# Dane-ME/keypoint-detection

Measured on AMD Instinct MI355X. Metric: images/sec @ 256x192 COCO-17 (MultiPersonKeypointModel.forward, given boxes), higher is better.
Workload: dtype fp32; 1 GPU; C2: batch 64/GPU, 256x192x3, 1 box/img, heatmap head + soft-argmax decode; model=MultiPersonKeypointModel (MobileNetV3-Small+FPN, HeatmapHead), global_batch=64, height=256, width=192, persons=1, precision=split, parallelism=dp1, streams_per_gpu=1, gather=False, gather_pipelined=False

## Files before the change

### keypoint-detection_amd/csrc/conv_glds.hip

```cpp
#include <algorithm>
#include <type_traits>

#include "kpd_common.h"
#include "kpd_kernels.h"
#include "conv_epilogue.h"
#include "kpd_dma.h"

namespace {

typedef _Float16 f16x8 __attribute__((ext_vector_type(8)));
typedef __attribute__((address_space(3))) void lds_void;

constexpr int BM = 256, NT = 512, ROWB = 128;
constexpr unsigned OOB = 0x80000000u;

__device__ __forceinline__ void stamp16(unsigned long long* st, int i, unsigned long long v = 0, int row = -1) {
  if (st && threadIdx.x == 0)
    st[(size_t)(row < 0 ? blockIdx.x : row) * 8 + i] = v ? v : __builtin_amdgcn_s_memrealtime();
}

__device__ __forceinline__ float dpp_xor1(float x) {
  return __int_as_float(__builtin_amdgcn_mov_dpp(__float_as_int(x), 0xB1, 0xF, 0xF, true));
}
__device__ __forceinline__ float dpp_xor2(float x) {
// ... 828 lines not shown
  const int c = (int)(i - px * c8n) * 8, n = (int)(px / hw);
  int a_f, a_l, P;
  fpn0x_exps(sc[(size_t)n * kAmaxStride], sc[(size_t)(N + n) * kAmaxStride], w_exp0, w_expE, &a_f, &a_l, &P);
  const float s = ldexpf(1.f, which ? a_l : a_f);
  const float4 u = *reinterpret_cast<const float4*>(in + px * cin + c);
  const float4 v = *reinterpret_cast<const float4*>(in + px * cin + c + 4);
  const float x[8] = {u.x, u.y, u.z, u.w, v.x, v.y, v.z, v.w};
  typedef _Float16 f16x8v __attribute__((ext_vector_type(8)));
  f16x8v hi, lo;
#pragma unroll
  for (int e = 0; e < 8; ++e) {
    const float xs = x[e] * s;
    hi[e] = (_Float16)xs;
    lo[e] = (_Float16)(xs - (float)hi[e]);
  }
  _Float16* o = out + px * 2 * cin + (c / G) * 2 * G + c % G;
  *reinterpret_cast<f16x8v*>(o) = hi;
  *reinterpret_cast<f16x8v*>(o + G) = lo;
}

constexpr int HP = kHmPitch, HPP = kHmRoiPos;
constexpr int HMS = 56;
constexpr int AWIN = 384;
template <int BMH>
constexpr int hm_awin() { return BMH + 128 <= AWIN ? AWIN : BMH + 128; }
template <int BMH>
constexpr int hm_epi_parts() { return BMH > 256 ? 2 : 1; }
template <int CIN, bool SPLIT>
constexpr int hm_nab() { return (CIN > 0 && (SPLIT ? CIN * 4 : CIN * 2) == 128) ? 1 : 2; }
template <int BMH>
constexpr int kh_epi_parts() { return BMH > 128 ? 2 : 1; }
template <int BN, int BMH>
constexpr int kh_epi_bytes() { return BMH / kh_epi_parts<BMH>() * ((BN + 4) + 68) * 4; }
template <int BN, int SB, int BMH, bool SPLIT, int TPS, int NW, int MODE, int NAB = 2>
constexpr int hmconv_lds_bytes() {
  constexpr int EMODE = MODE >= 0 ? MODE : (BN == 64 ? 1 : 0);
  constexpr int RING = NAB * hm_awin<BMH>() * ROWB + SB * BN * ROWB * TPS;
  constexpr int EPI = EMODE == 2 ? (BN == 128 ? kh_epi_bytes<BN, BMH>() : 0)
                      : EMODE != 0 && EMODE != 3 ? 0 : epi_lds_bytes<BMH / hm_epi_parts<BMH>(), 128, NW * 64>();
  return RING > EPI ? RING : EPI;
}

template <int BMH>
constexpr int hm_pst_stores() { return 2 * 2 * ((BMH / 2 + 31) / 32) * 2; }
template <int BN, int SB, int DBG, int BMH, bool SPLIT, int CIN, int TPS, bool DB, int NW, int MODE, int NTAP,
          bool PST = false>
__device__ __forceinline__ void hmconv_tile(const HmConvArgs& p, char* lds, const int L, const int m_off,
                                            const bool pre = false, const int next_m0 = -1) {
  constexpr int NTH = NW * 64;
  constexpr int EMODE = MODE >= 0 ? MODE : (BN == 64 ? 1 : 0);
  static_assert(NTAP == 9 || (NTAP == 10 && EMODE == 2 && SPLIT && !DB), "tenth tap: KH downsample");
  static_assert(EMODE != 2 || (SPLIT && !DB), "KH epilogue: split, single fragment set");
  constexpr int WAVES_N = BN / 64, WAVES_M = NW / WAVES_N;
  constexpr int WM = BMH / WAVES_M, FM = WM / 16, FN = 4;
  constexpr int AW = hm_awin<BMH>();
  static_assert(WM % 16 == 0 && BMH + 128 <= AW && AW % (8 * NW) == 0, "tile rows");
  static_assert(NW == 8 || (BN == 64 && SPLIT && DB), "4 waves: the conv 3 split DB variant only");
  constexpr int A_LD = AW / 8 / NW;
  static_assert(A_LD <= 9 || TPS > 1, "window pieces: one per tap");
  constexpr int B_LD = BN / 8 / NW;
  constexpr int ABUF = AW * ROWB, BSTAGE = BN * ROWB * TPS;
  static_assert(TPS == 1 || (SPLIT && NTAP % TPS == 0), "taps per step");
  constexpr bool FINAL = EMODE == 1;
  constexpr int NAB = hm_nab<CIN, SPLIT>();
  static_assert(hmconv_lds_bytes<BN, SB, BMH, SPLIT, TPS, NW, MODE, NAB>() <= 160 * 1024, "LDS budget");
  static_assert(!PST || NAB == 2, "persistent tiles: two window buffers");
  static_assert(!PST || (SPLIT && EMODE == 0 && SB == 2 && TPS == 1 && !DB && NW == 8 && NTAP == 9 && BN == 256 &&
                         BMH <= 224 && DBG == 0), "persistent tiles: split conv 1 / conv 2 (BN = cout = 256)");
  auto a_at = [&](int c) { return PST ? (c & 1) * (ABUF + BSTAGE) : NAB == 1 ? 0 : (c & 1) * ABUF; };
  auto b_at = [&](int st) { return PST ? st * (ABUF + BSTAGE) + ABUF : NAB * ABUF + st * BSTAGE; };

  int tid = threadIdx.x;
  if constexpr (PST) asm volatile("" : "+v"(tid));
  const int lane = tid & 63, wave = tid >> 6;
  const int wm = EMODE == 2 ? wave % WAVES_M : wave / WAVES_N, wn = EMODE == 2 ? wave / WAVES_M : wave % WAVES_N;
  const int NTL = p.cout / BN;
  const int m0 = HP + m_off + (L / NTL) * BMH, n0 = (L % NTL) * BN;
  if (m0 >= p.R * HPP) return;
  const int Mtot = p.R * HPP, cin = CIN ? CIN : p.cin, RB = SPLIT ? cin * 4 : cin * 2, NC = RB / 128, KT = NTAP * NC;
  stamp16(p.stamps, 0);
  const int wbase = max(m0 - 64, 0);
  const i32x4 rin = make_rsrc(static_cast<const char*>(p.in) + (size_t)wbase * RB,
                              (int)min(((long)Mtot - wbase) * RB, 0x7fffffffL));
  const i32x4 rwt = make_rsrc(p.wt, p.wt_bytes);
  const unsigned lds0 = (unsigned)reinterpret_cast<unsigned long long>((lds_void*)lds);
  const int lrow = lane >> 3, lchunk = (lane & 7) ^ lrow;
  unsigned a_off[A_LD];
#pragma unroll
// ... 90 lines not shown
  const int KS = KT / TPS;
  if (!PST || !pre) {
#pragma unroll
    for (int i = 0; i < A_LD; ++i) issue_a(0, i);
#pragma unroll
    for (int k = 0; k < SB - 1; ++k)
      if (k < KS) issue_b(k);
    barrier_k(KS < SB - 1);
  } else {
    if (p.amax_idx >= 0) wait_vmcnt<hm_pst_stores<224>() + 2>();
    else wait_vmcnt<hm_pst_stores<224>()>();
    __builtin_amdgcn_s_waitcnt(0xC07F);
    __builtin_amdgcn_s_barrier();
    asm volatile("" ::: "memory");
  }
  stamp16(p.stamps, 1);
  stamp16(p.stamps, 6, __builtin_amdgcn_s_memtime());
  auto issue_a_at = [&](int k1) {
    const int s1 = k1 * TPS, c1 = s1 / NTAP, jj = (s1 - c1 * NTAP) / TPS;
    if (c1 + 1 >= NC) return;
    if constexpr (TPS == 1) {
      if (jj < A_LD) issue_a(c1 + 1, jj);
    } else {
      constexpr int NST = 9 / TPS;
#pragma unroll
      for (int i = 0; i < A_LD; ++i)
        if (i >= jj * A_LD / NST && i < (jj + 1) * A_LD / NST) issue_a(c1 + 1, i);
    }
  };
  issue_a_at(0);
  if (SB - 1 < KS) issue_b(SB - 1);
  auto issue_at = [&](int k1) {
    if constexpr ((DBG & 2) == 0) {
      issue_a_at(k1);
      if (k1 + SB - 1 < KS) issue_b(k1 + SB - 1);
    }
  };
  if constexpr (!SPLIT) {
    Half f0, f1;
    load_half(0, 0, f0);
    for (int k = 0; k < KT; ++k) {
      load_half(k, 1, f1);
      __builtin_amdgcn_s_setprio(1);
      mma_half(f0);
      __builtin_amdgcn_s_setprio(0);
      if (k + 1 < KT) {
        const int k1 = k + 1;
        barrier_k(k1 + SB - 2 >= KT);
        issue_at(k1);
        load_half(k1, 0, f0);
// ... 10 lines not shown
      const int c = k / NTAP, t = k - c * NTAP, off = t == 9 ? 0 : (t / 3 - 1) * HP + (t % 3 - 1);
      const char* ab = lds + a_at(c);
      const int r0w = wm * WM + r16 + 64 + off;
      const int ach = (((q ? 4 : 0) + g) ^ (r0w & 7)) << 4;
#pragma unroll
      for (int i = 0; i < FM; ++i) f[i] = *reinterpret_cast<const uint4*>(ab + (r0w + i * 16) * ROWB + ach);
    };
    const bool late = p.stagger && __builtin_amdgcn_readfirstlane(wave) >= 4;
    auto pass = [&](f32x4 (&A)[FM][FN], const uint4* a, const uint4* b) {
      if constexpr ((DBG & 1) != 0) {
        A[0][0][0] += __uint_as_float(a[0].x ^ b[FN - 1].w);
        return;
      }
      __builtin_amdgcn_s_setprio(1);
#pragma unroll
      for (int i = 0; i < FM; ++i)
#pragma unroll
        for (int j = 0; j < FN; ++j)
          A[i][j] = __builtin_amdgcn_mfma_f32_16x16x32_f16(__builtin_bit_cast(f16x8, a[i]), __builtin_bit_cast(f16x8, b[j]),
                                                           A[i][j], 0, 0, 0);
      __builtin_amdgcn_s_setprio(0);
    };
    if constexpr (DB) {
      static_assert(SB == 2 && 9 % TPS == 0, "DB loop: 2-stage ring");
      int aoff[9];
#pragma unroll
      for (int t = 0; t < 9; ++t) {
        const int r0w = wm * WM + r16 + 64 + (t / 3 - 1) * HP + (t % 3 - 1);
        aoff[t] = r0w * ROWB + ((g ^ (r0w & 7)) << 4);
      }
      struct Frag { uint4 ah[FM], al[FM], bh[FN], bl[FN]; };
      auto rd_all = [&](int c, int t, int stage, Frag& f) {
        const char* ab = lds + a_at(c);
        const char* bb = lds + b_at(stage) + (t % TPS) * BN * ROWB + b_row;
#pragma unroll
        for (int i = 0; i < FM; ++i) {
          f.al[i] = *reinterpret_cast<const uint4*>(ab + (aoff[t] ^ 64) + i * 16 * ROWB);
          f.ah[i] = *reinterpret_cast<const uint4*>(ab + aoff[t] + i * 16 * ROWB);
        }
#pragma unroll
        for (int j = 0; j < FN; ++j) {
          f.bh[j] = *reinterpret_cast<const uint4*>(bb + j * 16 * ROWB + bch0);
          f.bl[j] = *reinterpret_cast<const uint4*>(bb + j * 16 * ROWB + bch1);
        }
      };
      Frag f0, f1;
      rd_all(0, 0, 0, f0);
      for (int c = 0; c < NC; c += 2) {
#pragma unroll
        for (int tt = 0; tt < 18; ++tt) {
          const int cc = c + tt / 9, t = tt % 9, k = cc * 9 + t;
          Frag& cur = (tt & 1) ? f1 : f0;
          Frag& nxt = (tt & 1) ? f0 : f1;
          pass(acc, cur.al, cur.bh);
          const bool kstep = k + 1 < KT && (t + 1) % TPS == 0;
          if (k + 1 < KT) {
            const int tn = (tt + 1) % 18, cn = c + (tt + 1) / 9;
            if (kstep) {
              const int k1 = (k + 1) / TPS;
              barrier_k(k1 + SB - 2 >= KS);
              if (!late) issue_at(k1);
            }
            rd_all(cn, tn % 9, ((tn / 9) * (9 / TPS) + (tn % 9) / TPS) & 1, nxt);
          }
          pass(acc, cur.ah, cur.bh);
          if (kstep && late) issue_at((k + 1) / TPS);
          pass(acc, cur.ah, cur.bl);
        }
      }
    } else {
    auto run_loop = [&](auto NBc, auto NMc, auto NM9c) {
      constexpr int NB_ = decltype(NBc)::value;
      auto rd_bn = [&](int k, int q, uint4* f) {
        const char* bb = lds + b_at((k / TPS) % SB) + (k % TPS) * BN * ROWB;
#pragma unroll
        for (int j = 0; j < NB_; ++j)
          f[j] = *reinterpret_cast<const uint4*>(bb + b_row + j * 16 * ROWB + (q ? bch1 : bch0));
      };
      auto passn = [&](f32x4 (&A)[FM][FN], const uint4* a, const uint4* b, auto NMx) {
        constexpr int NM_ = decltype(NMx)::value;
        if constexpr (NM_ == FN) {
          pass(A, a, b);
        } else if constexpr (NM_ > 0) {
          if constexpr ((DBG & 1) != 0) {
            A[0][0][0] += __uint_as_float(a[0].x ^ b[0].w);
            return;
// ... 442 lines not shown
            char* ob = static_cast<char*>(p.out) + (size_t)m * (p.ns * 4) + (co >> 5) * 128 + (co & 31) * 2;
            *reinterpret_cast<f16x4*>(ob) = hi;
            *reinterpret_cast<f16x4*>(ob + 64) = lo;
          } else {
            *reinterpret_cast<float4*>(p.outf + ((size_t)r * HMS * HMS + yy * HMS + xx) * p.nf +
                                       (co - p.ns)) = make_float4(o[0], o[1], o[2], o[3]);
          }
        }
      }
  
    }
  }
  if (p.stamps) {
    asm volatile("s_waitcnt vmcnt(0)" ::: "memory");
    stamp16(p.stamps, 3);
    stamp16(p.stamps, 5, (unsigned long long)KT);
  }
}

template <int BN, int SB, int DBG = 0, int BMH = BM, bool SPLIT = false, int CIN = 0, int TPS = 1, bool DB = false,
          int NW = 8, int MODE = -1, int NTAP = 9>
__global__ __launch_bounds__(NW * 64) void hmconv_kernel(const HmConvArgs p) {
  __shared__ __attribute__((aligned(1024))) char lds[hmconv_lds_bytes<BN, SB, BMH, SPLIT, TPS, NW, MODE,
                                                                      hm_nab<CIN, SPLIT>()>()];
  hmconv_tile<BN, SB, DBG, BMH, SPLIT, CIN, TPS, DB, NW, MODE, NTAP>(p, lds, xcd_remap(blockIdx.x, gridDim.x),
                                                                        p.m_off);
}

template <typename T>
__device__ __forceinline__ void kernarg_copy(T& dst) {
  typedef const __attribute__((address_space(4))) unsigned* KaPtr;
  KaPtr ka = (KaPtr)__builtin_amdgcn_kernarg_segment_ptr();
  asm volatile("" : "+s"(ka));
  static_assert(sizeof(T) % 4 == 0, "argument block");
  unsigned* d = reinterpret_cast<unsigned*>(&dst);
#pragma unroll
  for (int i = 0; i < (int)(sizeof(T) / 4); ++i) d[i] = ka[i];
}

template <int CIN>
__global__ __launch_bounds__(512) void hmconv_persist_kernel(const HmConvArgs p) {
  __shared__ __attribute__((aligned(1024))) char lds[hmconv_lds_bytes<256, 2, 224, true, 1, 8, -1>()];
  const int G = gridDim.x, w = xcd_remap(blockIdx.x, G);
  const int F = p.mix_F, H = p.mix_H, tail_off = p.m_off + F * 224;
  bool pre = false;
  for (int t = w; t < F; t += G) {
    HmConvArgs pl;
// ... 249 lines not shown
      m.mix_lead = ncu / 16;
      g = dim3((unsigned)(m.mix_F + m.mix_H));
    };
    if (fin && !dbg && !no_tail && !a.stamps && (!split || (a.cin == 256 && hm_db))) {
      const long nfull = rows / BM, F = nfull / ncu * ncu, rem = rows - F * BM, H = (rem + 127) / 128;
      if (split && mix_ok(F, H)) {
        HmConvArgs m = a;
        dim3 g;
        mix_set(m, F, H, g);
        hipLaunchKernelGGL((hmconv_mixed_kernel<64, 2, BM, 128, 256, 3, true, -1>), g, dim3(NT), 0, st, m);
        const hipError_t e = hipGetLastError();
        if (e != hipSuccess) return e;
        continue;
      }
      if (F > 0 && H > 0 && H <= ncu) {
        const dim3 g1((unsigned)F), g2((unsigned)H);
        HmConvArgs a2 = a;
        a2.m_off = (int)(F * BM);
        if (split && hm3_nw4) {
          hipLaunchKernelGGL((hmconv_kernel<64, 2, 0, BM, true, 256, 3, true, 4>), g1, dim3(256), 0, st, a);
          hipLaunchKernelGGL((hmconv_kernel<64, 2, 0, 128, true, 256, 3, true, 4>), g2, dim3(256), 0, st, a2);
        } else if (split) {
          hipLaunchKernelGGL((hmconv_kernel<64, 2, 0, BM, true, 256, 3, true>), g1, dim3(NT), 0, st, a);
          hipLaunchKernelGGL((hmconv_kernel<64, 2, 0, 128, true, 256, 3, true>), g2, dim3(NT), 0, st, a2);
        } else {
          hipLaunchKernelGGL((hmconv_kernel<64, 4>), g1, dim3(NT), 0, st, a);
          hipLaunchKernelGGL((hmconv_kernel<64, 4, 0, 128>), g2, dim3(NT), 0, st, a2);
        }
        const hipError_t e = hipGetLastError();
        if (e != hipSuccess) return e;
        continue;
      }
    }
    static const bool no_tail12 = kpd_diag_env("KPD_HM12_NOTAIL") != nullptr;
#if KPD_DIAG
    static const int persist_env = kpd_diag_env("KPD_HM_PERSIST") ? atoi(kpd_diag_env("KPD_HM_PERSIST")) : 0;
    if (split && !fin && bn == 256 && bm == 224 && a.cout == 256 && (a.cin == 64 || a.cin == 256) && !dbg &&
        !a.stamps && persist_env) {
      const long F = rows / 224 / ncu * ncu, rem = rows - F * 224, H = (rem + 191) / 192;
      if (F > 0 && H <= ncu && F + H < 0x7fffffffL / 224) {
        HmConvArgs m = a;
        m.mix_F = (int)F;
        m.mix_H = (int)H;
        if (a.cin == 64) hipLaunchKernelGGL((hmconv_persist_kernel<64>), dim3((unsigned)ncu), dim3(NT), 0, st, m);
        else hipLaunchKernelGGL((hmconv_persist_kernel<256>), dim3((unsigned)ncu), dim3(NT), 0, st, m);
        const hipError_t e = hipGetLastError();
        if (e != hipSuccess) return e;
// ... 184 lines not shown
```

### keypoint-detection_amd/csrc/head_kernels.hip

```cpp
#include <algorithm>

#include "kpd_common.h"
#include "kpd_kernels.h"

namespace {
constexpr int HM = 56;
static_assert(HM % 4 == 0, "hm_spool / hm_sapply take 4 pixels per load instruction");
constexpr int HMP = HM * HM;
constexpr int NK = 17;
constexpr int TOPK = 64;
constexpr int FC = 128;

__device__ __forceinline__ void slotmap_image(const float* __restrict__ boxes, int b, int P, int32_t* __restrict__ slot);
__global__ __launch_bounds__(256) void topk_kernel(const float* __restrict__ stats, int tiles, int HW,
                                                   const float* __restrict__ w0, const float* __restrict__ b0,
                                                   const float* __restrict__ w2, const float* __restrict__ b2,
                                                   int32_t* __restrict__ topk, float* __restrict__ scores_out,
                                                   const float* __restrict__ boxes, int P, int32_t* __restrict__ slot,
                                                   float* __restrict__ imax, float* __restrict__ sc_zero, int sc_n) {
  extern __shared__ __attribute__((aligned(16))) float tsm[];
  float* sw0 = tsm;
  float* sw2 = sw0 + 8 * FC;
  __shared__ float avg[FC], mx[FC], h[16], sc[FC];
  const int n = blockIdx.x, tid = threadIdx.x, c = tid;
// ... 610 lines not shown
      const float ov[4] = {o.x * ssc, o.y * ssc, o.z * ssc, o.w * ssc};
      f16x4 hi, lo;
#pragma unroll
      for (int e = 0; e < 4; ++e) {
        hi[e] = (_Float16)ov[e];
        lo[e] = (_Float16)(ov[e] - (float)hi[e]);
      }
      _Float16* ob = reinterpret_cast<_Float16*>(xs) + opix * 2 * TOPK + (c >> 3) * 64 + (c & 7) * 4;
      *reinterpret_cast<f16x4*>(ob) = hi;
      *reinterpret_cast<f16x4*>(ob + 32) = lo;
    } else if (out_bf16) {
      const size_t opix = out_bf16 == 2 ? hm_pos(r, y, px)
                                        : ((size_t)r * HM + y) * HM + px;
      bf16x4 ob;
      ob[0] = (__bf16)o.x; ob[1] = (__bf16)o.y; ob[2] = (__bf16)o.z; ob[3] = (__bf16)o.w;
      *reinterpret_cast<bf16x4*>(reinterpret_cast<__bf16*>(xs) + opix * TOPK + 4 * c) = ob;
    } else {
      reinterpret_cast<float4*>(reinterpret_cast<float*>(xs) + (((size_t)r * HM + y) * HM + px) * TOPK)[c] = o;
    }
  }
}

constexpr int kAttBR = 8;
__global__ __launch_bounds__(512) void hm_attn_kernel(const float* __restrict__ roi, const float* __restrict__ cw,
                                                      const float* __restrict__ saw, const float* __restrict__ sab,
                                                      void* __restrict__ xs, int out_bf16, const float* __restrict__ hsc,
                                                      int use_sp, float* __restrict__ sw_out) {
  constexpr int NI = HM / 4, BR = kAttBR, PR = BR + 6;
  __shared__ float w[98];
  __shared__ float2 pool[PR][HM + 6];
  __shared__ float ssw[BR][HM];
  const int nb = HM / BR;
  const int nblk = gridDim.x, L = blockIdx.x;
  const int qx = nblk / 8, rx = nblk % 8, x8 = L % 8, k8 = L / 8;
  const int g = (x8 < rx ? x8 * (qx + 1) : rx * (qx + 1) + (x8 - rx) * qx) + k8;
  const int r = g / nb, y0 = (g - r * nb) * BR;
  const int tid = threadIdx.x, lane = tid & 63, wave = tid >> 6, pp = lane >> 4, c = lane & 15;
  const float4 cq = reinterpret_cast<const float4*>(cw + (size_t)r * TOPK)[c];
  if (tid < 98) w[tid] = saw[tid];
  for (int i = tid; i < PR * 6; i += 512) {
    const int rr = i / 6, cc = i - rr * 6;
    pool[rr][cc < 3 ? cc : HM + cc] = make_float2(0.f, 0.f);
  }
  for (int pr = wave; pr < PR; pr += 8) {
    const int y = y0 - 3 + pr;
    if (y < 0 || y >= HM) {
      if (lane < HM) pool[pr][lane + 3] = make_float2(0.f, 0.f);
      continue;
    }
    const float4* src = reinterpret_cast<const float4*>(roi + ((size_t)r * HM + y) * HM * TOPK);
    float4 v[NI];
#pragma unroll
    for (int i = 0; i < NI; ++i) v[i] = src[(4 * i + pp) * (TOPK / 4) + c];
#pragma unroll
    for (int i = 0; i < NI; ++i) {
      const float a = v[i].x * cq.x, b = v[i].y * cq.y, cc = v[i].z * cq.z, d = v[i].w * cq.w;
      float sm = (a + b) + (cc + d), m = fmaxf(fmaxf(a, b), fmaxf(cc, d));
      sm += dpp_f<0xB1>(sm); m = fmaxf(m, dpp_f<0xB1>(m));
      sm += dpp_f<0x4E>(sm); m = fmaxf(m, dpp_f<0x4E>(m));
      sm += dpp_f<0x124>(sm); m = fmaxf(m, dpp_f<0x124>(m));
      sm += dpp_f<0x128>(sm); m = fmaxf(m, dpp_f<0x128>(m));
      if (c == 0) pool[pr][4 * i + pp + 3] = make_float2(sm / (float)TOPK, m);
    }
  }
  __syncthreads();
  if (tid < BR * HM) {
    const int j = tid / HM, x = tid - j * HM, y = y0 + j;
    float a = 0.f;
#pragma unroll
    for (int ky = 0; ky < 7; ++ky) {
      const int iy = y + ky - 3;
      if (iy < 0 || iy >= HM) continue;
#pragma unroll
      for (int kx = 0; kx < 7; ++kx) {
        const int ix = x + kx - 3;
        if (ix < 0 || ix >= HM) continue;
        const float2 sv2 = pool[j + ky][x + kx];
        a = fmaf(w[ky * 7 + kx], sv2.x, a);
        a = fmaf(w[49 + ky * 7 + kx], sv2.y, a);
      }
    }
    ssw[j][x] = use_sp ? kpd_sigmoid(a + sab[0]) : 1.f;
    if (sw_out) sw_out[((size_t)r * HM + y) * HM + x] = ssw[j][x];
  }
  const float ssc = out_bf16 == 3 ? ldexpf(1.f, split_exp_of(hsc[(size_t)r * 4])) : 1.f;
  __syncthreads();
  {
    const int j = wave, y = y0 + j;
    const float4* src = reinterpret_cast<const float4*>(roi + ((size_t)r * HM + y) * HM * TOPK);
    float4 v[NI];
#pragma unroll
    for (int i = 0; i < NI; ++i) v[i] = src[(4 * i + pp) * (TOPK / 4) + c];
#pragma unroll
    for (int i = 0; i < NI; ++i) {
      const int px = 4 * i + pp;
      const float sw = ssw[j][px];
      const float4 o = make_float4((v[i].x * cq.x) * sw, (v[i].y * cq.y) * sw, (v[i].z * cq.z) * sw, (v[i].w * cq.w) * sw);
      if (out_bf16 == 3) {
        const size_t opix = hm_pos(r, y, px);
        const float ov[4] = {o.x * ssc, o.y * ssc, o.z * ssc, o.w * ssc};
        f16x4 hi, lo;
#pragma unroll
        for (int e = 0; e < 4; ++e) {
          hi[e] = (_Float16)ov[e];
          lo[e] = (_Float16)(ov[e] - (float)hi[e]);
        }
        _Float16* ob = reinterpret_cast<_Float16*>(xs) + opix * 2 * TOPK + (c >> 3) * 64 + (c & 7) * 4;
        *reinterpret_cast<f16x4*>(ob) = hi;
        *reinterpret_cast<f16x4*>(ob + 32) = lo;
      } else if (out_bf16) {
        const size_t opix = out_bf16 == 2 ? hm_pos(r, y, px)
                                          : ((size_t)r * HM + y) * HM + px;
        bf16x4 ob;
        ob[0] = (__bf16)o.x; ob[1] = (__bf16)o.y; ob[2] = (__bf16)o.z; ob[3] = (__bf16)o.w;
        *reinterpret_cast<bf16x4*>(reinterpret_cast<__bf16*>(xs) + opix * TOPK + 4 * c) = ob;
      } else {
        reinterpret_cast<float4*>(reinterpret_cast<float*>(xs) + (((size_t)r * HM + y) * HM + px) * TOPK)[c] = o;
      }
    }
  }
}

__global__ __launch_bounds__(64) void hm_final_kernel(const float* __restrict__ h3, const float* __restrict__ w,
                                                      const float* __restrict__ b, const int32_t* __restrict__ slot,
                                                      int P, float* __restrict__ heat_out) {
  __shared__ float sw[NK * TOPK];
  __shared__ float sb[NK];
  const int y = blockIdx.x, r = blockIdx.y, x = threadIdx.x;
// ... 130 lines not shown
  const size_t lds = std::max<size_t>((size_t)cap * 4, kRoiKhLds);
  hipLaunchKernelGGL(roi_kh_kernel, dim3(HM, R), dim3(256), lds, st, feat, Hf, Wf, topk, boxes, P, roi, roi_stats,
                     cap, static_cast<const _Float16*>(w1s), w1_exp, b1, w2, b2, bound, bdiv, bstride, hsc,
                     static_cast<_Float16*>(out), stamps);
  return hipGetLastError();
}
hipError_t launch_hm_chattn(const float* roi_stats, int R, const float* w0, const float* b0, const float* w2,
                            const float* b2, float* cw, float* hsc, hipStream_t st, int abs_in) {
  hipLaunchKernelGGL(hm_chattn_kernel, dim3(R), dim3(64), 0, st, roi_stats, w0, b0, w2, b2, cw, hsc, abs_in);
  return hipGetLastError();
}
hipError_t launch_hm_spool(const float* roi, const float* cw, int R, float* smap, hipStream_t st) {
  hipLaunchKernelGGL(hm_spool_kernel, dim3(HM, R), dim3(64), 0, st, roi, cw, smap);
  return hipGetLastError();
}
hipError_t launch_hm_sapply(const float* roi, const float* cw, const float* smap, const float* saw,
                            const float* sab, int R, void* xs, int out_bf16, hipStream_t st, const float* hsc,
                            int use_sp, float* sw_out) {
  hipLaunchKernelGGL(hm_sapply_kernel, dim3(HM, R), dim3(64), 0, st, roi, cw, smap, saw, sab, xs, out_bf16, hsc,
                     use_sp, sw_out);
  return hipGetLastError();
}
hipError_t launch_hm_attn(const float* roi, const float* cw, const float* saw, const float* sab, int R, void* xs,
                          int out_bf16, hipStream_t st, const float* hsc, int use_sp, float* sw_out) {
  static_assert(HM % kAttBR == 0 && kAttBR == 8, "one wave per band row");
  if (R <= 0) return hipSuccess;
  hipLaunchKernelGGL(hm_attn_kernel, dim3((unsigned)(R * (HM / kAttBR))), dim3(512), 0, st, roi, cw, saw, sab, xs,
                     out_bf16, hsc, use_sp, sw_out);
  return hipGetLastError();
}
hipError_t launch_hm_final(const float* h3, int R, const float* w, const float* b, const int32_t* slot, int P,
                           float* heat_out, hipStream_t st) {
  hipLaunchKernelGGL(hm_final_kernel, dim3(HM, R), dim3(64), 0, st, h3, w, b, slot, P, heat_out);
  return hipGetLastError();
}
hipError_t launch_decode(const float* heat_out, const float* boxes, const int32_t* slot, int R, int P,
                         float* kpts_out, float* vis_out, hipStream_t st) {
  hipLaunchKernelGGL(decode_kernel, dim3(R, NK), dim3(64), 0, st, heat_out, boxes, slot, P, kpts_out, vis_out);
  return hipGetLastError();
}
```

### keypoint-detection_amd/csrc/kpd_kernels.h

```cpp
#pragma once
#include <hip/hip_runtime.h>
#include <stdint.h>
#include <vector>

struct ConvArgs {
  const void* in;
  const void* wt;
  const float* bias;
  void* out;
  const float* res;
  const float* a_scale;
  float* stats;
  int N, H, W;
  int cin_p, cout_p;
  int in_cstride, out_cstride;
  int rh, rw;
  int act;
  int M;
  int tiles_per_img;
  float* amax;
  const float* post_scale;
  const float* post_shift;
  int act2, act3;
  int in_bytes, wt_bytes;
// ... 202 lines not shown
size_t lateral_chain_lds_bytes(const LatChainArgs& a);
bool lateral_chain_ok(const LatChainArgs& a);
hipError_t launch_lateral_chain(const LatChainArgs& a, int N, hipStream_t st);
hipError_t launch_lateral_stream(const float* in, int cin_p, const float* w, const float* bias, const float* res,
                                 int N, int H, int W, int rh, int rw, void* out, hipStream_t st);

hipError_t launch_topk(const float* stats, int N, int tiles, int HW, const float* w0, const float* b0,
                       const float* w2, const float* b2, int32_t* topk, float* scores, hipStream_t st,
                       const float* boxes = nullptr, int P = 0, int32_t* slot = nullptr, float* imax = nullptr,
                       float* sc_zero = nullptr, int sc_n = 0);
hipError_t launch_slotmap(const float* boxes, int B, int P, int32_t* slot,
                          hipStream_t st);
hipError_t launch_roi_kh(const float* feat, int Hf, int Wf, const int32_t* topk, const float* boxes, int R, int P,
                        float* roi, float* roi_stats, const void* w1s, int w1_exp, const float* b1, const float* w2,
                        const float* b2, const float* bound, int bdiv, int bstride, float* hsc, void* out,
                        hipStream_t st, unsigned long long* stamps = nullptr);
hipError_t launch_roi_align(const float* feat, int Hf, int Wf, int Cf, const int32_t* topk,
                            const float* boxes, int R, int P, float* roi, float* roi_stats,
                            hipStream_t st, unsigned long long* stamps = nullptr);
hipError_t launch_hm_chattn(const float* roi_stats, int R, const float* w0, const float* b0,
                            const float* w2, const float* b2, float* cw, float* hsc, hipStream_t st,
                            int abs_in = 0);
hipError_t launch_hm_spool(const float* roi, const float* cw, int R, float* smap, hipStream_t st);
hipError_t launch_hm_attn(const float* roi, const float* cw, const float* saw, const float* sab, int R, void* xs,
                          int out_bf16, hipStream_t st, const float* hsc, int use_sp, float* sw_out);
hipError_t launch_hm_sapply(const float* roi, const float* cw, const float* smap, const float* saw,
                            const float* sab, int R, void* xs, int out_bf16, hipStream_t st,
                            const float* hsc = nullptr, int use_sp = 1, float* sw_out = nullptr);
hipError_t launch_hm_final(const float* h3, int R, const float* w, const float* b, const int32_t* slot,
                           int P, float* heat_out, hipStream_t st);
hipError_t launch_decode(const float* heat_out, const float* boxes, const int32_t* slot, int R, int P,
                         float* kpts_out, float* vis_out, hipStream_t st);

hipError_t launch_nms(const float* boxes, const float* scores, int n, float thr, int max_out,
                      int32_t* keep, int32_t* n_keep, void* scratch, size_t scratch_bytes, hipStream_t st);
hipError_t launch_nms_sets(const float* boxes, const float* scores, int sets, int n, float thr, int max_out,
                           int max_keep, int32_t* keep, int32_t* n_keep, void* scratch, hipStream_t st, int filter,
                           float* out_boxes, float* out_scores);
size_t nms_scratch_bytes(int n);

hipError_t launch_adaptive_pool56(const float* in, int B, int Hf, int Wf, int C, float* out, hipStream_t st);
bool person_detect_fits(int Wf);
hipError_t launch_person_detect(const float* feat, int B, int Hf, int Wf, const float* w, const float* bias,
                                const float* anchors, int img_h, int img_w, float conf, float* cand_boxes,
                                float* cand_scores, hipStream_t st);
hipError_t launch_person_decode(const float* head, int B, int hc, const float* anchors, int img_h, int img_w,
                                float conf, float* cand_boxes, float* cand_scores, hipStream_t st);
hipError_t launch_kh_att(float* x, const float* sa1, const float* w, const float* b, size_t npix, hipStream_t st);
// ... 135 lines not shown
```

### keypoint-detection_amd/csrc/kpd_plan.hip

```cpp
#include "kpd_plan_int.h"

namespace {
thread_local std::string g_err;
}

int fail(int code, const std::string& msg) {
  g_err = msg;
  return code;
}

int kpd_fail_einval(const char* msg) { return fail(KPD_EINVAL, msg); }
int kpd_fail_hip(hipError_t e, const char* where) {
  return fail(KPD_EHIP, std::string(where) + ": " + hipGetErrorString(e));
}

thread_local KpdPathLog* g_kpd_path = nullptr;

namespace {
struct PathRow { const char* name; unsigned sites; };
const PathRow kPathRows[KP_COUNT] = {
#define KPD_PATH_ROW(id, name, sites) {name, sites},
    KPD_PATH_TOKENS(KPD_PATH_ROW)
#undef KPD_PATH_ROW
};
// ... 359 lines not shown
  Work w;
  const size_t need = carve(p, d, nullptr, w);
  if (need > p->ws_bytes[k]) {
    if (p->ws[k]) HIP_TRY(hipFree(p->ws[k]));
    p->ws[k] = nullptr;
    HIP_TRY(hipMalloc(&p->ws[k], need));
    p->ws_bytes[k] = need;
  }
  carve(p, d, reinterpret_cast<char*>(p->ws[k]), p->work[k]);
  p->work[k].sc_dirty = true;
  ++p->ws_epoch;
  if (hm_padded(p)) HIP_TRY(hipMemsetAsync(p->ws[k], 0, need, st));
  p->dims[k] = d;
  p->have_work[k] = true;
  return KPD_OK;
}

static int run_heatmap_head(const Pass& ps, int R, int P, float* heat_out, int parts, float* sw_out,
                            unsigned long long* stamps2, unsigned long long* stamps3,
                            unsigned long long* stamps1 = nullptr, int abs_in = 0) {
  kpd_plan* p = ps.p; Work& w = *ps.w; const hipStream_t st = ps.st;
  std::unique_ptr<Stage> att_stage(new Stage(p, "hm_attention", st));
  const bool hsplit = p->precision == KPD_PRECISION_SPLIT;
  HIP_TRY(launch_hm_chattn(w.roi_stats, R, p->hca_w0, p->hca_b0, p->hca_w2, p->hca_b2, w.cw,
                           hsplit ? w.hsc : nullptr, st, abs_in));
  if (!(parts & KPD_HEAD_CHANNEL_ATT)) HIP_TRY(launch_fill(w.cw, (long)R * 64, 1.f, st));
  const bool bf = p->precision == KPD_PRECISION_MIXED;
  const int xs_mode = hsplit ? 3 : bf ? (hm_padded(p) ? 2 : 1) : 0;
  static const bool att_2k = kpd_diag_env("KPD_HM_ATT_2K") != nullptr;
  kpd_path(att_2k ? KP_HM_ATTN_2K : KP_HM_ATTN);
  if (att_2k) {
    HIP_TRY(launch_hm_spool(w.roi, w.cw, R, w.smap, st));
    HIP_TRY(launch_hm_sapply(w.roi, w.cw, w.smap, p->sa_w, p->sa_b, R, w.xs, xs_mode, st, w.hsc,
                             (parts & KPD_HEAD_SPATIAL_ATT) != 0, sw_out));
  } else {
    HIP_TRY(launch_hm_attn(w.roi, w.cw, p->sa_w, p->sa_b, R, w.xs, xs_mode, st, w.hsc,
                           (parts & KPD_HEAD_SPATIAL_ATT) != 0, sw_out));
  }
  att_stage.reset();
  if (!(parts & KPD_HEAD_CONVS)) return KPD_OK;
  const HmSplit sp1{w.hsc, 0.f, 1.f, 0, p->hm1.bc, p->hm1.bs, 0, 1};
  const HmSplit sp2{w.hsc, p->hm1.bc, p->hm1.bs, 0, p->hm2.bc, p->hm2.bs, 1, -1};
  const HmSplit sp3{w.hsc, p->hm2.bc, p->hm2.bs, 1, 0.f, 0.f, -1, -1};
  std::unique_ptr<Stage> c1(new Stage(p, "hm_conv1", st));
  if (int rc = hm_conv(ps, p->hm1, w.xs, R, 64, w.h1, 1, nullptr, stamps1, &sp1)) return rc;
  c1.reset();
  std::unique_ptr<Stage> c2(new Stage(p, "hm_conv2", st));
  if (int rc = hm_conv(ps, p->hm2, w.h1, R, p->hm1.cout_p, w.h2, 1, nullptr, stamps2, &sp2)) return rc;
  c2.reset();
  std::unique_ptr<Stage> c3(new Stage(p, "hm_conv3", st));
  static const bool no_fin_fuse = kpd_diag_env("KPD_NO_FINAL_FUSE") != nullptr;
  const bool fin_fused = (p->hm3.bf16 || p->hm3.ws) && p->hm3.cout_p == 64 && (!no_fin_fuse || p->hm3.ws);
  const HmFinal fin{p->fin_w, p->fin_b, w.slot, P, heat_out};
  if (int rc = hm_conv(ps, p->hm3, w.h2, R, p->hm2.cout_p, w.h3, 2, fin_fused ? &fin : nullptr, stamps3, &sp3))
    return rc;
  c3.reset();
  kpd_path(fin_fused ? KP_HM_FINAL_FUSED : KP_HM_FINAL);
  if (!fin_fused) HIP_TRY(launch_hm_final(w.h3, R, p->fin_w, p->fin_b, w.slot, P, heat_out, st));
  return KPD_OK;
}
// ... 1223 lines not shown
```

Before: 42110 images/s.

## Fold channel attention into spatial attention kernel and add 64-row conv3 tail variant

Fuses the channel-attention MLP into the spatial-attention kernel so each block recomputes the per-ROI channel weights from the ROI statistics, removing a separate launch and the dependency on it. The attention kernel also loads each band row once into registers and reuses it for both pooling and output, instead of reading ROI rows twice, and it now splits halo rows per wave. Separately, the conv3 tail gets a 64-row, 4-wave, 3-stage weight-ring variant with a tighter LDS window when the tail fits in one wave of CUs. The trade-offs are redundant per-block MLP work, higher register pressure, and a more intricate pipeline schedule.

```diff
diff --git a/keypoint-detection_amd/csrc/conv_glds.hip b/keypoint-detection_amd/csrc/conv_glds.hip
--- a/keypoint-detection_amd/csrc/conv_glds.hip
+++ b/keypoint-detection_amd/csrc/conv_glds.hip
@@ -874,8 +874,10 @@
 constexpr int HP = kHmPitch, HPP = kHmRoiPos;
 constexpr int HMS = 56;
 constexpr int AWIN = 384;
-template <int BMH>
-constexpr int hm_awin() { return BMH + 128 <= AWIN ? AWIN : BMH + 128; }
+template <int BMH, bool TIGHT = false>
+constexpr int hm_awin() { return !TIGHT && BMH + 128 <= AWIN ? AWIN : BMH + 128; }
+template <bool SPLIT, bool DB, int SB>
+constexpr bool hm_tight() { return SPLIT && DB && SB > 2; }
 template <int BMH>
 constexpr int hm_epi_parts() { return BMH > 256 ? 2 : 1; }
 template <int CIN, bool SPLIT>
@@ -884,10 +886,10 @@
 constexpr int kh_epi_parts() { return BMH > 128 ? 2 : 1; }
 template <int BN, int BMH>
 constexpr int kh_epi_bytes() { return BMH / kh_epi_parts<BMH>() * ((BN + 4) + 68) * 4; }
-template <int BN, int SB, int BMH, bool SPLIT, int TPS, int NW, int MODE, int NAB = 2>
+template <int BN, int SB, int BMH, bool SPLIT, int TPS, int NW, int MODE, int NAB = 2, bool TIGHT = false>
 constexpr int hmconv_lds_bytes() {
   constexpr int EMODE = MODE >= 0 ? MODE : (BN == 64 ? 1 : 0);
-  constexpr int RING = NAB * hm_awin<BMH>() * ROWB + SB * BN * ROWB * TPS;
+  constexpr int RING = NAB * hm_awin<BMH, TIGHT>() * ROWB + SB * BN * ROWB * TPS;
   constexpr int EPI = EMODE == 2 ? (BN == 128 ? kh_epi_bytes<BN, BMH>() : 0)
                       : EMODE != 0 && EMODE != 3 ? 0 : epi_lds_bytes<BMH / hm_epi_parts<BMH>(), 128, NW * 64>();
   return RING > EPI ? RING : EPI;
@@ -905,7 +907,8 @@
   static_assert(EMODE != 2 || (SPLIT && !DB), "KH epilogue: split, single fragment set");
   constexpr int WAVES_N = BN / 64, WAVES_M = NW / WAVES_N;
   constexpr int WM = BMH / WAVES_M, FM = WM / 16, FN = 4;
-  constexpr int AW = hm_awin<BMH>();
+  constexpr bool TIGHT = hm_tight<SPLIT, DB, SB>();
+  constexpr int AW = hm_awin<BMH, TIGHT>();
   static_assert(WM % 16 == 0 && BMH + 128 <= AW && AW % (8 * NW) == 0, "tile rows");
   static_assert(NW == 8 || (BN == 64 && SPLIT && DB), "4 waves: the conv 3 split DB variant only");
   constexpr int A_LD = AW / 8 / NW;
@@ -915,7 +918,7 @@
   static_assert(TPS == 1 || (SPLIT && NTAP % TPS == 0), "taps per step");
   constexpr bool FINAL = EMODE == 1;
   constexpr int NAB = hm_nab<CIN, SPLIT>();
-  static_assert(hmconv_lds_bytes<BN, SB, BMH, SPLIT, TPS, NW, MODE, NAB>() <= 160 * 1024, "LDS budget");
+  static_assert(hmconv_lds_bytes<BN, SB, BMH, SPLIT, TPS, NW, MODE, NAB, TIGHT>() <= 160 * 1024, "LDS budget");
   static_assert(!PST || NAB == 2, "persistent tiles: two window buffers");
   static_assert(!PST || (SPLIT && EMODE == 0 && SB == 2 && TPS == 1 && !DB && NW == 8 && NTAP == 9 && BN == 256 &&
                          BMH <= 224 && DBG == 0), "persistent tiles: split conv 1 / conv 2 (BN = cout = 256)");
@@ -1052,10 +1055,11 @@
     if constexpr (TPS == 1) {
       if (jj < A_LD) issue_a(c1 + 1, jj);
     } else {
-      constexpr int NST = 9 / TPS;
+      constexpr int NST = 9 / TPS - (SB - 2);
+      static_assert(NST >= 1, "window pieces: before the next chunk's first weights");
 #pragma unroll
       for (int i = 0; i < A_LD; ++i)
-        if (i >= jj * A_LD / NST && i < (jj + 1) * A_LD / NST) issue_a(c1 + 1, i);
+        if (jj < NST && i >= jj * A_LD / NST && i < (jj + 1) * A_LD / NST) issue_a(c1 + 1, i);
     }
   };
   issue_a_at(0);
@@ -1112,7 +1116,8 @@
       __builtin_amdgcn_s_setprio(0);
     };
     if constexpr (DB) {
-      static_assert(SB == 2 && 9 % TPS == 0, "DB loop: 2-stage ring");
+      constexpr int UC = 2, NSUB = UC * 9;
+      static_assert(9 % TPS == 0 && (UC * (9 / TPS)) % SB == 0, "DB loop: whole turns of the weight ring per iteration");
       int aoff[9];
 #pragma unroll
       for (int t = 0; t < 9; ++t) {
@@ -1136,22 +1141,22 @@
       };
       Frag f0, f1;
       rd_all(0, 0, 0, f0);
-      for (int c = 0; c < NC; c += 2) {
-#pragma unroll
-        for (int tt = 0; tt < 18; ++tt) {
+      for (int c = 0; c < NC; c += UC) {
+#pragma unroll
+        for (int tt = 0; tt < NSUB; ++tt) {
           const int cc = c + tt / 9, t = tt % 9, k = cc * 9 + t;
           Frag& cur = (tt & 1) ? f1 : f0;
           Frag& nxt = (tt & 1) ? f0 : f1;
           pass(acc, cur.al, cur.bh);
           const bool kstep = k + 1 < KT && (t + 1) % TPS == 0;
           if (k + 1 < KT) {
-            const int tn = (tt + 1) % 18, cn = c + (tt + 1) / 9;
+            const int tn = (tt + 1) % NSUB, cn = c + (tt + 1) / 9;
             if (kstep) {
               const int k1 = (k + 1) / TPS;
               barrier_k(k1 + SB - 2 >= KS);
               if (!late) issue_at(k1);
             }
-            rd_all(cn, tn % 9, ((tn / 9) * (9 / TPS) + (tn % 9) / TPS) & 1, nxt);
+            rd_all(cn, tn % 9, ((tn / 9) * (9 / TPS) + (tn % 9) / TPS) % SB, nxt);
           }
           pass(acc, cur.ah, cur.bh);
           if (kstep && late) issue_at((k + 1) / TPS);
@@ -1640,7 +1645,7 @@
           int NW = 8, int MODE = -1, int NTAP = 9>
 __global__ __launch_bounds__(NW * 64) void hmconv_kernel(const HmConvArgs p) {
   __shared__ __attribute__((aligned(1024))) char lds[hmconv_lds_bytes<BN, SB, BMH, SPLIT, TPS, NW, MODE,
-                                                                      hm_nab<CIN, SPLIT>()>()];
+                                                                      hm_nab<CIN, SPLIT>(), hm_tight<SPLIT, DB, SB>()>()];
   hmconv_tile<BN, SB, DBG, BMH, SPLIT, CIN, TPS, DB, NW, MODE, NTAP>(p, lds, xcd_remap(blockIdx.x, gridDim.x),
                                                                         p.m_off);
 }
@@ -1936,7 +1941,12 @@
           hipLaunchKernelGGL((hmconv_kernel<64, 2, 0, 128, true, 256, 3, true, 4>), g2, dim3(256), 0, st, a2);
         } else if (split) {
           hipLaunchKernelGGL((hmconv_kernel<64, 2, 0, BM, true, 256, 3, true>), g1, dim3(NT), 0, st, a);
-          hipLaunchKernelGGL((hmconv_kernel<64, 2, 0, 128, true, 256, 3, true>), g2, dim3(NT), 0, st, a2);
+          static const bool tail128 = kpd_diag_env("KPD_HM3_TAIL128") != nullptr;
+          const long H64 = (rem + 63) / 64;
+          if (!tail128 && H64 <= ncu)
+            hipLaunchKernelGGL((hmconv_kernel<64, 3, 0, 64, true, 256, 3, true, 4>), dim3((unsigned)H64), dim3(256), 0,
+                               st, a2);
+          else hipLaunchKernelGGL((hmconv_kernel<64, 2, 0, 128, true, 256, 3, true>), g2, dim3(NT), 0, st, a2);
         } else {
           hipLaunchKernelGGL((hmconv_kernel<64, 4>), g1, dim3(NT), 0, st, a);
           hipLaunchKernelGGL((hmconv_kernel<64, 4, 0, 128>), g2, dim3(NT), 0, st, a2);
diff --git a/keypoint-detection_amd/csrc/head_kernels.hip b/keypoint-detection_amd/csrc/head_kernels.hip
--- a/keypoint-detection_amd/csrc/head_kernels.hip
+++ b/keypoint-detection_amd/csrc/head_kernels.hip
@@ -656,46 +656,142 @@
 }
 
 constexpr int kAttBR = 8;
-__global__ __launch_bounds__(512) void hm_attn_kernel(const float* __restrict__ roi, const float* __restrict__ cw,
+__device__ __forceinline__ void wave_lds_sync() {
+  __builtin_amdgcn_fence(__ATOMIC_RELEASE, "wavefront");
+  __builtin_amdgcn_wave_barrier();
+  __builtin_amdgcn_fence(__ATOMIC_ACQUIRE, "wavefront");
+}
+template <bool FOLD>
+__global__ __launch_bounds__(512, 4) void hm_attn_kernel(const float* __restrict__ roi, const float* __restrict__ cw,
                                                       const float* __restrict__ saw, const float* __restrict__ sab,
                                                       void* __restrict__ xs, int out_bf16, const float* __restrict__ hsc,
-                                                      int use_sp, float* __restrict__ sw_out) {
+                                                      int use_sp, float* __restrict__ sw_out,
+                                                      const float* __restrict__ roi_stats, const float* __restrict__ w0,
+                                                      const float* __restrict__ b0, const float* __restrict__ w2,
+                                                      const float* __restrict__ b2, float* __restrict__ cw_out,
+                                                      float* __restrict__ hsc_out) {
   constexpr int NI = HM / 4, BR = kAttBR, PR = BR + 6;
   __shared__ float w[98];
   __shared__ float2 pool[PR][HM + 6];
   __shared__ float ssw[BR][HM];
+  __shared__ float scw[TOPK], savg[TOPK], smx[TOPK], sh[8], su0;
+  __shared__ float sst[FOLD ? HM * 2 * TOPK : 1], sw0[FOLD ? 4 * TOPK : 1];
   const int nb = HM / BR;
   const int nblk = gridDim.x, L = blockIdx.x;
   const int qx = nblk / 8, rx = nblk % 8, x8 = L % 8, k8 = L / 8;
   const int g = (x8 < rx ? x8 * (qx + 1) : rx * (qx + 1) + (x8 - rx) * qx) + k8;
   const int r = g / nb, y0 = (g - r * nb) * BR;
   const int tid = threadIdx.x, lane = tid & 63, wave = tid >> 6, pp = lane >> 4, c = lane & 15;
-  const float4 cq = reinterpret_cast<const float4*>(cw + (size_t)r * TOPK)[c];
+  const int jb = wave >= 3 ? wave - 3 : wave + 5;
+  const int ph = wave < 3 ? wave : wave + 8, yh = y0 - 3 + ph;
+  const bool halo = ph < PR && yh >= 0 && yh < HM;
+  constexpr int NST = HM * 2 * TOPK / 512;
+  static_assert(HM * 2 * TOPK % 512 == 0, "statistics per thread");
+  float stv[FOLD ? NST : 1], w0v = 0.f, b0v = 0.f, b2v = 0.f;
+  float4 w2v = make_float4(0.f, 0.f, 0.f, 0.f);
+  if constexpr (FOLD) {
+    if (tid < 4 * TOPK) w0v = w0[tid];
+    if (wave == 7) {
+      w2v = reinterpret_cast<const float4*>(w2)[lane];
+      b2v = b2[lane];
+      b0v = b0[lane & 3];
+    }
+    const float* st = roi_stats + (size_t)r * HM * 2 * TOPK;
+#pragma unroll
+    for (int u = 0; u < NST; ++u) stv[u] = st[tid + 512 * u];
+  }
+  constexpr int NH = NI / 2;
+  float4 vb[NI], vh[NH];
+  const float4* srch = reinterpret_cast<const float4*>(roi + ((size_t)r * HM + (halo ? yh : 0)) * HM * TOPK);
+  {
+    const float4* src = reinterpret_cast<const float4*>(roi + ((size_t)r * HM + y0 + jb) * HM * TOPK);
+#pragma unroll
+    for (int i = 0; i < NI; ++i) vb[i] = src[(4 * i + pp) * (TOPK / 4) + c];
+  }
+  if constexpr (FOLD) {
+#pragma unroll
+    for (int u = 0; u < NST; ++u) sst[tid + 512 * u] = stv[u];
+    if (tid < 4 * TOPK) sw0[tid] = w0v;
+  }
+  if (halo) {
+#pragma unroll
+    for (int i = 0; i < NH; ++i) vh[i] = srch[(4 * i + pp) * (TOPK / 4) + c];
+  }
+  float4 cq;
+  if constexpr (!FOLD) cq = reinterpret_cast<const float4*>(cw + (size_t)r * TOPK)[c];
   if (tid < 98) w[tid] = saw[tid];
   for (int i = tid; i < PR * 6; i += 512) {
     const int rr = i / 6, cc = i - rr * 6;
     pool[rr][cc < 3 ? cc : HM + cc] = make_float2(0.f, 0.f);
   }
-  for (int pr = wave; pr < PR; pr += 8) {
-    const int y = y0 - 3 + pr;
-    if (y < 0 || y >= HM) {
-      if (lane < HM) pool[pr][lane + 3] = make_float2(0.f, 0.f);
-      continue;
-    }
-    const float4* src = reinterpret_cast<const float4*>(roi + ((size_t)r * HM + y) * HM * TOPK);
-    float4 v[NI];
-#pragma unroll
-    for (int i = 0; i < NI; ++i) v[i] = src[(4 * i + pp) * (TOPK / 4) + c];
-#pragma unroll
-    for (int i = 0; i < NI; ++i) {
-      const float a = v[i].x * cq.x, b = v[i].y * cq.y, cc = v[i].z * cq.z, d = v[i].w * cq.w;
-      float sm = (a + b) + (cc + d), m = fmaxf(fmaxf(a, b), fmaxf(cc, d));
-      sm += dpp_f<0xB1>(sm); m = fmaxf(m, dpp_f<0xB1>(m));
-      sm += dpp_f<0x4E>(sm); m = fmaxf(m, dpp_f<0x4E>(m));
-      sm += dpp_f<0x124>(sm); m = fmaxf(m, dpp_f<0x124>(m));
-      sm += dpp_f<0x128>(sm); m = fmaxf(m, dpp_f<0x128>(m));
-      if (c == 0) pool[pr][4 * i + pp + 3] = make_float2(sm / (float)TOPK, m);
-    }
+  if constexpr (FOLD) {
+    __syncthreads();
+    if (wave == 7) {
+      float s = 0.f, m = -INFINITY;
+#pragma unroll 4
+      for (int row = 0; row < HM; ++row) {
+        s += sst[row * 2 * TOPK + lane];
+        m = fmaxf(m, sst[row * 2 * TOPK + TOPK + lane]);
+      }
+      savg[lane] = s / (float)HMP;
+      smx[lane] = m;
+      const float u0 = fmaxf(wave_max(m), 0.f);
+      if (lane == 0) {
+        su0 = u0;
+        if (hsc_out && y0 == 0) {
+          hsc_out[(size_t)r * 4] = u0;
+          hsc_out[(size_t)r * 4 + 1] = 0.f;
+        }
+      }
+      wave_lds_sync();
+      if (lane < 8) {
+        const int j = lane & 3;
+        const float* v = (lane < 4) ? savg : smx;
+        float a = b0v;
+#pragma unroll 8
+        for (int k = 0; k < TOPK; ++k) a = fmaf(sw0[j * TOPK + k], v[k], a);
+        sh[lane] = fmaxf(a, 0.f);
+      }
+      wave_lds_sync();
+      const float w2e[4] = {w2v.x, w2v.y, w2v.z, w2v.w};
+      float oa = b2v, om = b2v;
+#pragma unroll
+      for (int j = 0; j < 4; ++j) {
+        oa = fmaf(w2e[j], sh[j], oa);
+        om = fmaf(w2e[j], sh[4 + j], om);
+      }
+      const float cv = kpd_sigmoid(oa + om);
+      scw[lane] = cv;
+      if (y0 == 0) cw_out[(size_t)r * TOPK + lane] = cv;
+    }
+    __syncthreads();
+    cq = reinterpret_cast<const float4*>(scw)[c];
+  }
+  auto pool_px = [&](const float4& v, int pr, int i) {
+#pragma clang fp contract(off)
+    const float a = v.x * cq.x, b = v.y * cq.y, cc = v.z * cq.z, d = v.w * cq.w;
+    float sm = fmaf(v.x, cq.x, b) + fmaf(v.z, cq.z, d), m = fmaxf(fmaxf(a, b), fmaxf(cc, d));
+    sm += dpp_f<0xB1>(sm); m = fmaxf(m, dpp_f<0xB1>(m));
+    sm += dpp_f<0x4E>(sm); m = fmaxf(m, dpp_f<0x4E>(m));
+    sm += dpp_f<0x124>(sm); m = fmaxf(m, dpp_f<0x124>(m));
+    sm += dpp_f<0x128>(sm); m = fmaxf(m, dpp_f<0x128>(m));
+    if (c == 0) pool[pr][4 * i + pp + 3] = make_float2(sm / (float)TOPK, m);
+  };
+  if (halo) {
+    float4 v2[NH];
+#pragma unroll
+    for (int i = 0; i < NH; ++i) {
+      pool_px(vh[i], ph, i);
+      v2[i] = srch[(4 * (NH + i) + pp) * (TOPK / 4) + c];
+    }
+#pragma unroll
+    for (int i = 0; i < NI; ++i) pool_px(vb[i], 3 + jb, i);
+#pragma unroll
+    for (int i = 0; i < NH; ++i) pool_px(v2[i], ph, NH + i);
+  } else {
+#pragma unroll
+    for (int i = 0; i < NI; ++i) pool_px(vb[i], 3 + jb, i);
+    if (ph < PR && lane < HM) pool[ph][lane + 3] = make_float2(0.f, 0.f);
   }
   __syncthreads();
   if (tid < BR * HM) {
@@ -717,27 +813,26 @@
     ssw[j][x] = use_sp ? kpd_sigmoid(a + sab[0]) : 1.f;
     if (sw_out) sw_out[((size_t)r * HM + y) * HM + x] = ssw[j][x];
   }
-  const float ssc = out_bf16 == 3 ? ldexpf(1.f, split_exp_of(hsc[(size_t)r * 4])) : 1.f;
+  float ssc = 1.f;
+  if (out_bf16 == 3) ssc = ldexpf(1.f, split_exp_of(FOLD ? su0 : hsc[(size_t)r * 4]));
   __syncthreads();
   {
-    const int j = wave, y = y0 + j;
-    const float4* src = reinterpret_cast<const float4*>(roi + ((size_t)r * HM + y) * HM * TOPK);
-    float4 v[NI];
-#pragma unroll
-    for (int i = 0; i < NI; ++i) v[i] = src[(4 * i + pp) * (TOPK / 4) + c];
+    const int j = jb, y = y0 + j;
 #pragma unroll
     for (int i = 0; i < NI; ++i) {
       const int px = 4 * i + pp;
       const float sw = ssw[j][px];
-      const float4 o = make_float4((v[i].x * cq.x) * sw, (v[i].y * cq.y) * sw, (v[i].z * cq.z) * sw, (v[i].w * cq.w) * sw);
+      const float4 o = make_float4((vb[i].x * cq.x) * sw, (vb[i].y * cq.y) * sw, (vb[i].z * cq.z) * sw,
+                                   (vb[i].w * cq.w) * sw);
       if (out_bf16 == 3) {
+#pragma clang fp contract(off)
         const size_t opix = hm_pos(r, y, px);
-        const float ov[4] = {o.x * ssc, o.y * ssc, o.z * ssc, o.w * ssc};
+        const float oe[4] = {o.x, o.y, o.z, o.w};
         f16x4 hi, lo;
 #pragma unroll
         for (int e = 0; e < 4; ++e) {
-          hi[e] = (_Float16)ov[e];
-          lo[e] = (_Float16)(ov[e] - (float)hi[e]);
+          hi[e] = (_Float16)(oe[e] * ssc);
+          lo[e] = (_Float16)fmaf(oe[e], ssc, -(float)hi[e]);
         }
         _Float16* ob = reinterpret_cast<_Float16*>(xs) + opix * 2 * TOPK + (c >> 3) * 64 + (c & 7) * 4;
         *reinterpret_cast<f16x4*>(ob) = hi;
@@ -914,11 +1009,19 @@
   return hipGetLastError();
 }
 hipError_t launch_hm_attn(const float* roi, const float* cw, const float* saw, const float* sab, int R, void* xs,
-                          int out_bf16, hipStream_t st, const float* hsc, int use_sp, float* sw_out) {
+                          int out_bf16, hipStream_t st, const float* hsc, int use_sp, float* sw_out,
+                          const HmChAttFold* fold) {
   static_assert(HM % kAttBR == 0 && kAttBR == 8, "one wave per band row");
   if (R <= 0) return hipSuccess;
-  hipLaunchKernelGGL(hm_attn_kernel, dim3((unsigned)(R * (HM / kAttBR))), dim3(512), 0, st, roi, cw, saw, sab, xs,
-                     out_bf16, hsc, use_sp, sw_out);
+  const dim3 grid((unsigned)(R * (HM / kAttBR)));
+  if (fold) {
+    if (!fold->roi_stats || !fold->cw_out || (out_bf16 == 3 && !fold->hsc_out)) return hipErrorInvalidValue;
+    hipLaunchKernelGGL(hm_attn_kernel<true>, grid, dim3(512), 0, st, roi, cw, saw, sab, xs, out_bf16, hsc, use_sp,
+                       sw_out, fold->roi_stats, fold->w0, fold->b0, fold->w2, fold->b2, fold->cw_out, fold->hsc_out);
+  } else {
+    hipLaunchKernelGGL(hm_attn_kernel<false>, grid, dim3(512), 0, st, roi, cw, saw, sab, xs, out_bf16, hsc, use_sp,
+                       sw_out, nullptr, nullptr, nullptr, nullptr, nullptr, nullptr, nullptr);
+  }
   return hipGetLastError();
 }
 hipError_t launch_hm_final(const float* h3, int R, const float* w, const float* b, const int32_t* slot, int P,
diff --git a/keypoint-detection_amd/csrc/kpd_kernels.h b/keypoint-detection_amd/csrc/kpd_kernels.h
--- a/keypoint-detection_amd/csrc/kpd_kernels.h
+++ b/keypoint-detection_amd/csrc/kpd_kernels.h
@@ -248,8 +248,13 @@
                             const float* w2, const float* b2, float* cw, float* hsc, hipStream_t st,
                             int abs_in = 0);
 hipError_t launch_hm_spool(const float* roi, const float* cw, int R, float* smap, hipStream_t st);
+struct HmChAttFold {
+  const float *roi_stats, *w0, *b0, *w2, *b2;
+  float *cw_out, *hsc_out;
+};
 hipError_t launch_hm_attn(const float* roi, const float* cw, const float* saw, const float* sab, int R, void* xs,
-                          int out_bf16, hipStream_t st, const float* hsc, int use_sp, float* sw_out);
+                          int out_bf16, hipStream_t st, const float* hsc, int use_sp, float* sw_out,
+                          const HmChAttFold* fold = nullptr);
 hipError_t launch_hm_sapply(const float* roi, const float* cw, const float* smap, const float* saw,
                             const float* sab, int R, void* xs, int out_bf16, hipStream_t st,
                             const float* hsc = nullptr, int use_sp = 1, float* sw_out = nullptr);
diff --git a/keypoint-detection_amd/csrc/kpd_plan.hip b/keypoint-detection_amd/csrc/kpd_plan.hip
--- a/keypoint-detection_amd/csrc/kpd_plan.hip
+++ b/keypoint-detection_amd/csrc/kpd_plan.hip
@@ -405,20 +405,24 @@
   kpd_plan* p = ps.p; Work& w = *ps.w; const hipStream_t st = ps.st;
   std::unique_ptr<Stage> att_stage(new Stage(p, "hm_attention", st));
   const bool hsplit = p->precision == KPD_PRECISION_SPLIT;
-  HIP_TRY(launch_hm_chattn(w.roi_stats, R, p->hca_w0, p->hca_b0, p->hca_w2, p->hca_b2, w.cw,
-                           hsplit ? w.hsc : nullptr, st, abs_in));
+  static const bool att_2k = kpd_diag_env("KPD_HM_ATT_2K") != nullptr;
+  static const bool ca_sep = kpd_diag_env("KPD_HM_CHATT_SEP") != nullptr;
+  const bool ca_fold = (parts & KPD_HEAD_CHANNEL_ATT) && !abs_in && !att_2k && !ca_sep;
+  if (!ca_fold)
+    HIP_TRY(launch_hm_chattn(w.roi_stats, R, p->hca_w0, p->hca_b0, p->hca_w2, p->hca_b2, w.cw,
+                             hsplit ? w.hsc : nullptr, st, abs_in));
   if (!(parts & KPD_HEAD_CHANNEL_ATT)) HIP_TRY(launch_fill(w.cw, (long)R * 64, 1.f, st));
   const bool bf = p->precision == KPD_PRECISION_MIXED;
   const int xs_mode = hsplit ? 3 : bf ? (hm_padded(p) ? 2 : 1) : 0;
-  static const bool att_2k = kpd_diag_env("KPD_HM_ATT_2K") != nullptr;
   kpd_path(att_2k ? KP_HM_ATTN_2K : KP_HM_ATTN);
   if (att_2k) {
     HIP_TRY(launch_hm_spool(w.roi, w.cw, R, w.smap, st));
     HIP_TRY(launch_hm_sapply(w.roi, w.cw, w.smap, p->sa_w, p->sa_b, R, w.xs, xs_mode, st, w.hsc,
                              (parts & KPD_HEAD_SPATIAL_ATT) != 0, sw_out));
   } else {
+    const HmChAttFold fold{w.roi_stats, p->hca_w0, p->hca_b0, p->hca_w2, p->hca_b2, w.cw, hsplit ? w.hsc : nullptr};
     HIP_TRY(launch_hm_attn(w.roi, w.cw, p->sa_w, p->sa_b, R, w.xs, xs_mode, st, w.hsc,
-                           (parts & KPD_HEAD_SPATIAL_ATT) != 0, sw_out));
+                           (parts & KPD_HEAD_SPATIAL_ATT) != 0, sw_out, ca_fold ? &fold : nullptr));
   }
   att_stage.reset();
   if (!(parts & KPD_HEAD_CONVS)) return KPD_OK;
```

After: 42330 images/s, median of 6. Within noise of the previous version (+0.5%).
